# someone-in-somewhere/multimodal_rag

Hardware: AMD Instinct MI355X
Metric: chunks embedded/sec + queries/sec top_k=5 over 1M×768 at 1/2/4/8 GPUs (higher is better)
Workload: dtype f16

## Files before the change

multimodal_rag_amd/csrc/encoder.hip:

```cpp
#include "mmrag_internal.h"
#include "tile_dma.h"

#include <atomic>
#include <chrono>
#include <type_traits>

#include <limits.h>
#include <stdlib.h>

using namespace mmrag;

namespace mmrag_impl {

constexpr float NEG_INF_F = -__builtin_inff();
typedef _Float16 half2_t __attribute__((ext_vector_type(2)));
__device__ inline float2 h2f(half2_t t) { return make_float2((float)t[0], (float)t[1]); }
__device__ inline half2_t f2h(float a, float b) {
    half2_t r;
    r[0] = (_Float16)a;
    r[1] = (_Float16)b;
    return r;
}

__device__ inline float wave_sum(float v) {
// ... 795 lines not shown
            const int c = wave + i * NWAVES;
            vreg[i] = make_uint4(0, 0, 0, 0);
            if (c < CH && k0 + lane < len) vreg[i] = *(const uint4 *)(Vp + (size_t)(k0 + lane) * ld + c * 8);
        }
    };
    auto store_tile_from = [&](int buf, const uint4(&kreg)[K_ITERS], const uint4(&vreg)[V_ITERS]) {
        char *kb = smem + buf * (K_BYTES + V_BYTES);
        char *vb = kb + K_BYTES;
#pragma unroll
        for (int i = 0; i < K_ITERS; ++i) {
            const int idx = threadIdx.x + i * NT;
            const int key = idx / CH, c = idx % CH;
            if (idx < KT * CH) {
                const int cs = DH == 64 ? (c ^ ((key >> 1) & 7)) : (c ^ ((key >> 2) & 3));
                *(uint4 *)(kb + key * KROW + cs * 16) = kreg[i];
            }
        }
#pragma unroll
        for (int i = 0; i < V_ITERS; ++i) {
            const int c = wave + i * NWAVES;
            if (c < CH) {
                const unsigned w[4] = {vreg[i].x, vreg[i].y, vreg[i].z, vreg[i].w};
#pragma unroll
                for (int e = 0; e < 8; ++e) {
                    const unsigned short bits = (unsigned short)(w[e >> 1] >> ((e & 1) * 16));
                    *(unsigned short *)(vb + (c * 8 + e) * VROW + lane * 2) = bits;
                }
            }
        }
    };

    f32x16_t o[NDB];
#pragma unroll
    for (int d = 0; d < NDB; ++d)
#pragma unroll
        for (int j = 0; j < 16; ++j) o[d][j] = 0.f;
    float m_run = NEG_INF_F, l_run = 0.f;

    auto load_tile = [&](int kt) { load_tile_into(kt, kreg0, vreg0); };
    auto store_tile = [&](int buf) { store_tile_from(buf, kreg0, vreg0); };
    if constexpr (RESIDENT) {
        uint4 kr[MAXT - 1][K_ITERS], vr[MAXT - 1][V_ITERS];
        load_tile(0);
#pragma unroll
        for (int t = 1; t < MAXT; ++t)
            if (t < n_tiles) load_tile_into(t, kr[t - 1], vr[t - 1]);
        store_tile(0);
#pragma unroll
        for (int t = 1; t < MAXT; ++t)
            if (t < n_tiles) store_tile_from(t, kr[t - 1], vr[t - 1]);
    } else {
        load_tile(0);
        store_tile(0);
    }
    __syncthreads();
    for (int kt = 0; kt < n_tiles; ++kt) {
        const int buf = RESIDENT ? kt : (kt & 1);
        if constexpr (!RESIDENT)
            if (kt + 1 < n_tiles) load_tile(kt + 1);
        const char *kb = smem + buf * (K_BYTES + V_BYTES);
        const char *vb = kb + K_BYTES;

        f32x16_t s[2];
#pragma unroll
        for (int b = 0; b < 2; ++b) {
#pragma unroll
            for (int j = 0; j < 16; ++j) s[b][j] = 0.f;
            const int key = b * 32 + r32;
#pragma unroll
            for (int ks = 0; ks < NQK; ++ks) {
                const int c = 2 * ks + hh;
                const int cs = DH == 64 ? (c ^ ((key >> 1) & 7)) : (c ^ ((key >> 2) & 3));
                const half8_t kf = *(const half8_t *)(kb + key * KROW + cs * 16);
                s[b] = __builtin_amdgcn_mfma_f32_32x32x16_f16(kf, qf[ks], s[b], 0, 0, 0);
            }
        }
        const int k0 = kt * KT;
        const bool edge = (k0 + KT > len) || (causal && k0 + KT - 1 > q_tile0 + wave * 32);
        if (edge) {
#pragma unroll
            for (int b = 0; b < 2; ++b)
#pragma unroll
                for (int j = 0; j < 16; ++j) {
                    const int key = k0 + b * 32 + (j & 3) + 8 * (j >> 2) + 4 * hh;
                    const bool ok = key < len && (!causal || key <= qi);
                    s[b][j] = ok ? s[b][j] : NEG_INF_F;
                }
        }
        float m_tile = NEG_INF_F;
#pragma unroll
        for (int b = 0; b < 2; ++b)
#pragma unroll
            for (int j = 0; j < 16; j += 2) m_tile = fmaxf(m_tile, fmaxf(s[b][j], s[b][j + 1]));
        m_tile = fmaxf(m_tile, __shfl_xor(m_tile, 32));
        const float m_new = fmaxf(m_run, m_tile);
        const float m_use = m_new == NEG_INF_F ? 0.f : m_new;
        const float c2 = scale * 1.4426950408889634f;
        const float mc = m_use * c2;
        const float alpha = __builtin_amdgcn_exp2f(m_run * c2 - mc);
        float psum = 0.f;
        half8_t pf[2][2];
#pragma unroll
        for (int b = 0; b < 2; ++b)
#pragma unroll
            for (int j = 0; j < 16; ++j) {
                const float pv = __builtin_amdgcn_exp2f(fmaf(s[b][j], c2, -mc));
                psum += pv;
                pf[b][j >> 3][j & 7] = (_Float16)pv;
            }
        l_run = l_run * alpha + psum;
        m_run = m_new;
#pragma unroll
        for (int d = 0; d < NDB; ++d)
#pragma unroll
            for (int j = 0; j < 16; ++j) o[d][j] *= alpha;
#pragma unroll
        for (int d = 0; d < NDB; ++d) {
            const char *vrow = vb + (d * 32 + r32) * VROW;
#pragma unroll
            for (int b = 0; b < 2; ++b)
#pragma unroll
                for (int st = 0; st < 2; ++st) {
                    const int kk = b * 32 + st * 16 + 4 * hh;
                    const half4_t lo = *(const half4_t *)(vrow + kk * 2);
                    const half4_t hi = *(const half4_t *)(vrow + (kk + 8) * 2);
                    half8_t vf;
#pragma unroll
                    for (int i = 0; i < 4; ++i) {
                        vf[i] = lo[i];
                        vf[4 + i] = hi[i];
                    }
                    o[d] = __builtin_amdgcn_mfma_f32_32x32x16_f16(vf, pf[b][st], o[d], 0, 0, 0);
                }
        }
        if constexpr (!RESIDENT) {
            if (kt + 1 < n_tiles) store_tile(buf ^ 1);
            __syncthreads();
        }
    }

    const float l_tot = l_run + __shfl_xor(l_run, 32);
    const float inv = l_tot > 0.f ? 1.0f / l_tot : 0.f;
    if (qi < len) {
        _Float16 *dst = ctx + (size_t)(seq0 + qi) * H + head * DH;
#pragma unroll
        for (int d = 0; d < NDB; ++d)
#pragma unroll
            for (int g = 0; g < 4; ++g) {
                half4_t v;
#pragma unroll
                for (int i = 0; i < 4; ++i) v[i] = (_Float16)(o[d][4 * g + i] * inv);
                *(half4_t *)(dst + d * 32 + 8 * g + 4 * hh) = v;
            }
    }
#endif
}

template <typename OutT>
__global__ __launch_bounds__(256) void pool_norm_kernel(const _Float16 *__restrict__ x,
                                                         const int *__restrict__ cu_seqlens,
                                                         const int *__restrict__ sel, OutT *__restrict__ out,
                                                         int H, int pool, int normalize) {
    __shared__ float red[4];
    const int b = blockIdx.x;
    const int s0 = cu_seqlens[b], s1 = cu_seqlens[b + 1];
    float vals[4];
    float sq = 0.f;
#pragma unroll
    for (int i = 0; i < 4; ++i) {
        const int c = threadIdx.x + i * 256;
        float v = 0.f;
        if (c < H) {
            if (pool == 0) {
                for (int t = s0; t < s1; ++t) v += (float)x[(size_t)t * H + c];
                const float cnt = (float)(s1 - s0);
                v = v / fmaxf(cnt, 1e-9f);
            } else {
                const int t = pool == 1 ? s0 : s0 + sel[b];
                v = (float)x[(size_t)t * H + c];
            }
        }
        vals[i] = v;
        sq += v * v;
    }
    sq = wave_sum(sq);
    if ((threadIdx.x & 63) == 0) red[threadIdx.x >> 6] = sq;
    __syncthreads();
    const float nrm = sqrtf(red[0] + red[1] + red[2] + red[3]);
    const float inv = normalize ? 1.0f / fmaxf(nrm, 1e-12f) : 1.0f;
#pragma unroll
    for (int i = 0; i < 4; ++i) {
        const int c = threadIdx.x + i * 256;
        if (c < H) out[(size_t)b * H + c] = (OutT)(vals[i] * inv);
    }
}

__global__ __launch_bounds__(256) void patchify_kernel(const void *__restrict__ pixels, int kind,
                                                        _Float16 *__restrict__ patches, int B, int IMG, int P) {
    const int G = IMG / P, NP = G * G, PK = 3 * P * P, CH = PK / 8;
    const long long total = (long long)B * NP * CH;
    const long long i = (long long)blockIdx.x * blockDim.x + threadIdx.x;
    if (i >= total) return;
    const int ch = (int)(i % CH);
    const long long prow = i / CH;
    const int pidx = (int)(prow % NP), b = (int)(prow / NP);
    const int e0 = ch * 8;
    const int c = e0 / (P * P), ph = (e0 / P) % P, pw = e0 % P;
    const int y = (pidx / G) * P + ph, x0 = (pidx % G) * P + pw;
    half8_t o;
    if (kind == MMRAG_PIXELS_F16_CHW) {
        o = *(const half8_t *)((const _Float16 *)pixels + (((size_t)b * 3 + c) * IMG + y) * IMG + x0);
    } else {
        const float mean[3] = {0.48145466f, 0.4578275f, 0.40821073f};
        const float stdv[3] = {0.26862954f, 0.26130258f, 0.27577711f};
        const unsigned char *src = (const unsigned char *)pixels + (((size_t)b * IMG + y) * IMG + x0) * 3 + c;
#pragma unroll
        for (int e = 0; e < 8; ++e) o[e] = (_Float16)(((float)src[e * 3] / 255.0f - mean[c]) / stdv[c]);
    }
    *(half8_t *)(patches + (size_t)prow * PK + e0) = o;
}

__global__ __launch_bounds__(256) void vit_assemble_ln_kernel(const _Float16 *__restrict__ emb,
                                                               const _Float16 *__restrict__ cls,
                                                               const _Float16 *__restrict__ pos,
                                                               const float *__restrict__ g, const float *__restrict__ b,
                                                               _Float16 *__restrict__ out, int T, int H, int S,
                                                               float eps) {
    const int lane = threadIdx.x & 63;
    const int row = blockIdx.x * 4 + (threadIdx.x >> 6);
    if (row >= T) return;
    const int t = row % S, img = row / S;
    const _Float16 *src = t == 0 ? cls : emb + ((size_t)img * (S - 1) + (t - 1)) * H;
    ln_row<2>(src, out + (size_t)row * H, g, b, H, eps, lane, pos + (size_t)t * H);
}

__global__ __launch_bounds__(256) void normalize_rows_kernel(const _Float16 *__restrict__ x, float *__restrict__ out,
                                                              int B, int D) {
    const int lane = threadIdx.x & 63;
    const int row = blockIdx.x * 4 + (threadIdx.x >> 6);
    if (row >= B) return;
    float sq = 0.f;
    for (int c = lane; c < D; c += 64) {
        const float v = (float)x[(size_t)row * D + c];
        sq += v * v;
    }
    const float inv = 1.0f / fmaxf(sqrtf(wave_sum(sq)), 1e-12f);
    for (int c = lane; c < D; c += 64) out[(size_t)row * D + c] = (float)x[(size_t)row * D + c] * inv;
}

template <int NWC>
__global__ __launch_bounds__(64 * NWC) void linear_small_kernel(const LinearParams p) {
#if defined(__HIP_DEVICE_COMPILE__)
    __shared__ float part[NWC][16][64];
    const int lane = threadIdx.x & 63;
    const int wave = threadIdx.x >> 6;
    const int r32 = lane & 31, h = lane >> 5;
    const int f0 = blockIdx.x * 32;
    const int kw = p.K / NWC;
    const int k_lo = wave * kw;
    const int fr = f0 + r32 < p.N ? f0 + r32 : p.N - 1;
    const _Float16 *wrow = (const _Float16 *)p.wt + (size_t)fr * p.K + k_lo + 8 * h;
    for (int t0 = 0; t0 < p.M; t0 += 32) {
        const int tr = t0 + r32 < p.M ? t0 + r32 : p.M - 1;
        const _Float16 *xrow = (const _Float16 *)p.x + (size_t)tr * p.K + k_lo + 8 * h;
        f32x16_t acc;
#pragma unroll
        for (int j = 0; j < 16; ++j) acc[j] = 0.0f;
        for (int k = 0; k < kw; k += 64) {
            half8_t a[4], b[4];
#pragma unroll
            for (int s_ = 0; s_ < 4; ++s_) {
                const bool in = k + 16 * s_ < kw;
                a[s_] = *(const half8_t *)(wrow + (in ? k + 16 * s_ : 0));
                b[s_] = *(const half8_t *)(xrow + (in ? k + 16 * s_ : 0));
            }
#pragma unroll
            for (int s_ = 0; s_ < 4; ++s_)
                if (k + 16 * s_ < kw) acc = __builtin_amdgcn_mfma_f32_32x32x16_f16(a[s_], b[s_], acc, 0, 0, 0);
        }
        if (t0 > 0) __syncthreads();
#pragma unroll
        for (int j = 0; j < 16; ++j) part[wave][j][lane] = acc[j];
        __syncthreads();
        const int g = wave & 3;
        const int t = t0 + r32;
        const int f = f0 + 8 * g + 4 * h;
        float v[4] = {0.f, 0.f, 0.f, 0.f};
        if (wave < 4) {
#pragma unroll
            for (int w = 0; w < NWC; ++w)
#pragma unroll
                for (int i = 0; i < 4; ++i) v[i] += part[w][4 * g + i][lane];
        }
        if (wave < 4 && t < p.M && f < p.N) {
            if (p.bias != nullptr) {
                const float4 bv = *(const float4 *)(p.bias + f);
                v[0] += bv.x, v[1] += bv.y, v[2] += bv.z, v[3] += bv.w;
            }
            half4_t o;
            if (p.act == MMRAG_ACT_GELU) {
#pragma unroll
                for (int i = 0; i < 4; ++i) o[i] = (_Float16)act_apply<MMRAG_ACT_GELU>(v[i]);
            } else if (p.act == MMRAG_ACT_QUICK_GELU) {
#pragma unroll
                for (int i = 0; i < 4; ++i) o[i] = (_Float16)act_apply<MMRAG_ACT_QUICK_GELU>(v[i]);
            } else {
// ... 136 lines not shown
    float2 *ln_stats_out = nullptr;
    const float2 *res_stats = nullptr;
    const float *res_gamma = nullptr, *res_beta = nullptr;
};

static bool takes_small16_kernel(long long M, int K, bool ln_in) {
    if (M > 64 || (debug_flags() & (DBG_LINEAR_NO_SMALL | DBG_LINEAR_SMALL32))) return false;
    if (ln_in) return K == 384 || K == 512 || K == 768 || K == 1024;
    return K == 384 || K == 512 || K == 768 || K == 1024 || K == 1536 || K == 2048 || K == 3072;
}

int launch_linear(const void *x, int M, int K, const void *wt, int N, const float *bias, int act,
                  const void *resid, void *out, hipStream_t s, const SmallNorms *norms = nullptr) {
    LinearParams p;
    p.ln_gamma = p.ln_beta = nullptr, p.ln_eps = 0.f, p.ln_stats_out = nullptr;
    p.res_stats = nullptr, p.res_gamma = p.res_beta = nullptr;
    if (norms != nullptr) {
        if (!takes_small16_kernel(M, K, norms->ln_gamma != nullptr)) {
            set_error("linear: folded LayerNorm needs the 16-feature single-query kernel (M=%d K=%d)", M, K);
            return MMRAG_EUNSUPPORTED;
        }
        p.ln_gamma = norms->ln_gamma, p.ln_beta = norms->ln_beta, p.ln_eps = norms->ln_eps, p.ln_stats_out = norms->ln_stats_out;
        p.res_stats = norms->res_stats, p.res_gamma = norms->res_gamma, p.res_beta = norms->res_beta;
    }
    p.x = (const char *)x;
    p.wt = (const char *)wt;
    p.bias = bias;
    p.resid = (const _Float16 *)resid;
    p.out = (_Float16 *)out;
    p.M = M, p.N = N, p.K = K, p.act = act;
    const unsigned dbg = debug_flags();
    p.xcd_order = (dbg & DBG_LINEAR_PLAIN) ? 0 : 1;
    p.dbg = dbg;
    if (M <= 64 && !(dbg & (DBG_LINEAR_NO_SMALL | DBG_LINEAR_SMALL32))) {
        const unsigned g16 = (unsigned)((N + 15) / 16);
        bool done = true;
        if (p.ln_gamma != nullptr) {
            if (K == 384) linear_small16_kernel<12, 1, true><<<g16, 768, 0, s>>>(p);
            else if (K == 512) linear_small16_kernel<16, 1, true><<<g16, 1024, 0, s>>>(p);
            else if (K == 768) linear_small16_kernel<12, 2, true><<<g16, 768, 0, s>>>(p);
            else linear_small16_kernel<16, 2, true><<<g16, 1024, 0, s>>>(p);
        } else if (K == 384) linear_small16_kernel<12, 1><<<g16, 768, 0, s>>>(p);
        else if (K == 512) linear_small16_kernel<16, 1><<<g16, 1024, 0, s>>>(p);
        else if (K == 768) linear_small16_kernel<12, 2><<<g16, 768, 0, s>>>(p);
        else if (K == 1024) linear_small16_kernel<16, 2><<<g16, 1024, 0, s>>>(p);
        else if (K == 1536) linear_small16_kernel<16, 3><<<g16, 1024, 0, s>>>(p);
        else if (K == 2048) linear_small16_kernel<16, 4><<<g16, 1024, 0, s>>>(p);
        else if (K == 3072) linear_small16_kernel<16, 6><<<g16, 1024, 0, s>>>(p);
        else done = false;
        if (done) return MMRAG_OK;
    }
    if (M <= 64 && (K / 4) % 16 == 0 && !(dbg & DBG_LINEAR_NO_SMALL)) {
        const unsigned g = (unsigned)((N + 31) / 32);
        if (K % 256 == 0) linear_small_kernel<16><<<g, 1024, 0, s>>>(p);
        else if (K % 128 == 0) linear_small_kernel<8><<<g, 512, 0, s>>>(p);
        else linear_small_kernel<4><<<g, 256, 0, s>>>(p);
        return MMRAG_OK;
    }
    const int cus = num_cus();
    const long long big_tiles = (long long)((M + 255) / 256) * ((N + 255) / 256);
    const long long tiles_f = (N + 255) / 256;
    const bool big_pays = (double)N >= 0.65 * (double)(tiles_f * 256);
    if (big_tiles >= cus && big_pays) {
        if (dbg & DBG_LINEAR_PLAIN)
            linear_kernel<256, 256, 4, 4, 2><<<(unsigned)big_tiles, 1024, 0, s>>>(p);
        else if (K >= 128 && N % 2 == 0 && !(dbg & DBG_LINEAR_NO_PERSIST)) {
            const unsigned grid = (unsigned)(big_tiles < cus ? big_tiles : cus);
            if (!(dbg & DBG_LINEAR_MFMA32) && N % 4 == 0) linear_persistent_kernel<2, 4, 16><<<grid, 512, 0, s>>>(p, (int)big_tiles, (int)tiles_f);
            else linear_persistent_kernel<2, 4, 32><<<grid, 512, 0, s>>>(p, (int)big_tiles, (int)tiles_f);
        } else
            linear_kernel<256, 256, 4, 4, 2, true><<<(unsigned)big_tiles, 1024, 0, s>>>(p);
    } else {
        const long long tiles = (long long)((M + 127) / 128) * ((N + 127) / 128);
        if ((dbg & DBG_LINEAR_TILE64) || (!(dbg & DBG_LINEAR_TILE128) && tiles < cus / 2)) {
            const long long t64 = (long long)((M + 63) / 64) * ((N + 63) / 64);
            linear_kernel<64, 64, 1, 1, 2, true><<<(unsigned)t64, 64, 0, s>>>(p);
            return MMRAG_OK;
        }
        linear_kernel<128, 128, 2, 2, 2, true><<<(unsigned)tiles, 256, 0, s>>>(p);
    }
    return MMRAG_OK;
}

}
using namespace mmrag_impl;

static std::atomic<long long> g_last_forward_us{0};

extern "C" {

int mmrag_linear_f16(const void *x, int64_t M, int K, const void *wt, int N, const float *bias, int act,
                     const void *resid, void *out, void *stream) {
    MMRAG_CHECK_ARG(x && wt && out, "linear: null pointer");
    MMRAG_CHECK_ARG(M > 0 && M < INT_MAX && N > 0 && K > 0, "linear: bad shape M=%lld N=%d K=%d", (long long)M, N, K);
    MMRAG_CHECK_ARG(K % 64 == 0, "linear: K=%d must be a multiple of 64 (128-byte fp16 slabs)", K);
    MMRAG_CHECK_ARG(N % 4 == 0, "linear: N=%d must be a multiple of 4", N);
    MMRAG_CHECK_ARG(act >= 0 && act <= 2, "linear: bad activation %d", act);
    MMRAG_CHECK_ARG(((uintptr_t)x % 16) == 0 && ((uintptr_t)wt % 16) == 0 && ((uintptr_t)out % 8) == 0 &&
                        ((uintptr_t)resid % 8) == 0 && ((uintptr_t)bias % 16) == 0,
                    "linear: misaligned pointer");
    launch_linear(x, (int)M, K, wt, N, bias, act, resid, out, (hipStream_t)stream);
    MMRAG_CHECK_HIP(hipGetLastError());
    return MMRAG_OK;
}

int mmrag_internal_linear_f16_norms(const void *x, int64_t M, int K, const void *wt, int N, const float *bias, int act,
                                    const void *resid, void *out, const float *ln_gamma, const float *ln_beta,
                                    float ln_eps, float *ln_stats_out, const float *res_stats, const float *res_gamma,
                                    const float *res_beta, void *stream) {
    MMRAG_CHECK_ARG(x && wt && out, "linear_norms: null pointer");
    MMRAG_CHECK_ARG(M > 0 && M <= 64 && N > 0 && N % 4 == 0, "linear_norms: bad shape M=%lld N=%d", (long long)M, N);
    MMRAG_CHECK_ARG(act >= 0 && act <= 2, "linear_norms: bad activation %d", act);
    MMRAG_CHECK_ARG((ln_gamma == nullptr) == (ln_beta == nullptr), "linear_norms: ln_gamma / ln_beta both or neither");
    MMRAG_CHECK_ARG(res_stats == nullptr || (resid && res_gamma && res_beta), "linear_norms: res_stats needs resid, res_gamma, res_beta");
    MMRAG_CHECK_ARG(((uintptr_t)x % 16) == 0 && ((uintptr_t)wt % 16) == 0 && ((uintptr_t)out % 8) == 0 &&
                        ((uintptr_t)resid % 8) == 0 && ((uintptr_t)bias % 16) == 0 && ((uintptr_t)ln_gamma % 16) == 0 &&
                        ((uintptr_t)ln_beta % 16) == 0 && ((uintptr_t)ln_stats_out % 8) == 0 &&
                        ((uintptr_t)res_stats % 8) == 0 && ((uintptr_t)res_gamma % 16) == 0 &&
                        ((uintptr_t)res_beta % 16) == 0,
                    "linear_norms: misaligned pointer");
    SmallNorms n;
    n.ln_gamma = ln_gamma, n.ln_beta = ln_beta, n.ln_eps = ln_eps, n.ln_stats_out = (float2 *)ln_stats_out;
    n.res_stats = (const float2 *)res_stats, n.res_gamma = res_gamma, n.res_beta = res_beta;
    const int st = launch_linear(x, (int)M, K, wt, N, bias, act, resid, out, (hipStream_t)stream, &n);
    if (st != MMRAG_OK) return st;
    MMRAG_CHECK_HIP(hipGetLastError());
    return MMRAG_OK;
}

int mmrag_layernorm_f16(const void *x, void *out, const float *gamma, const float *beta, int64_t T, int H,
                        float eps, void *stream) {
    MMRAG_CHECK_ARG(x && out && gamma && beta, "layernorm: null pointer");
    MMRAG_CHECK_ARG(T > 0 && H > 0 && H % 8 == 0 && H <= 1024, "layernorm: bad shape T=%lld H=%d (H % 8 == 0, <= 1024)", (long long)T, H);
    MMRAG_CHECK_ARG(((uintptr_t)x % 16) == 0 && ((uintptr_t)out % 16) == 0 && ((uintptr_t)gamma % 16) == 0 && ((uintptr_t)beta % 16) == 0, "layernorm: pointers must be 16-byte aligned");
    layernorm_kernel<<<(unsigned)((T + 3) / 4), 256, 0, (hipStream_t)stream>>>(
        (const _Float16 *)x, (_Float16 *)out, gamma, beta, (int)T, H, eps);
    MMRAG_CHECK_HIP(hipGetLastError());
    return MMRAG_OK;
}

int mmrag_embed_ln_f16(const int32_t *ids, const int32_t *pos_ids, const void *tok, const void *pos,
                       const void *type0, const float *gamma, const float *beta, void *out, int64_t T, int H,
                       int vocab, int max_pos, float eps, void *stream) {
    MMRAG_CHECK_ARG(ids && pos_ids && tok && pos && out, "embed_ln: null pointer");
    MMRAG_CHECK_ARG((gamma == nullptr) == (beta == nullptr), "embed_ln: gamma/beta must both be given or both null");
    MMRAG_CHECK_ARG(T > 0 && H > 0 && H % 8 == 0 && H <= 1024, "embed_ln: bad shape T=%lld H=%d", (long long)T, H);
    embed_ln_kernel<<<(unsigned)((T + 3) / 4), 256, 0, (hipStream_t)stream>>>(
        ids, pos_ids, (const _Float16 *)tok, (const _Float16 *)pos, (const _Float16 *)type0, gamma, beta,
        (_Float16 *)out, (int)T, H, vocab, max_pos, eps);
    MMRAG_CHECK_HIP(hipGetLastError());
    return MMRAG_OK;
}

int mmrag_attention_f16(const void *qkv, const int32_t *cu_seqlens, void *ctx, int B, int max_len, int H,
                        int n_heads, int causal, void *stream) {
    MMRAG_CHECK_ARG(qkv && cu_seqlens && ctx, "attention: null pointer");
    MMRAG_CHECK_ARG(B > 0 && max_len > 0 && n_heads > 0 && H % n_heads == 0, "attention: bad shape");
    const int dh = H / n_heads;
    MMRAG_CHECK_ARG(dh == 32 || dh == 64, "attention: head dim %d unsupported (32 or 64)", dh);
    MMRAG_CHECK_ARG(((uintptr_t)qkv % 16) == 0 && ((uintptr_t)ctx % 8) == 0, "attention: misaligned pointer");
    const dim3 grid((unsigned)((max_len + 127) / 128), (unsigned)n_heads, (unsigned)B);
    const float scale = 1.0f / sqrtf((float)dh);
    if (dh == 64 && max_len <= 256 && max_len > 128 && !(debug_flags() & DBG_ATTENTION_STREAMED)) {
        const dim3 grid8((unsigned)((max_len + 255) / 256), (unsigned)n_heads, (unsigned)B);
        attention_kernel<64, 2, true, 8><<<grid8, 512, 0, (hipStream_t)stream>>>((const _Float16 *)qkv, cu_seqlens,
                                                                                 (_Float16 *)ctx, H, scale, causal);
    } else if (dh == 64 && max_len > 256 && max_len <= 512 && !(debug_flags() & DBG_ATTENTION_STREAMED)) {
        const dim3 grid16((unsigned)((max_len + 511) / 512), (unsigned)n_heads, (unsigned)B);
        attention_kernel<64, 1, true, 16, 8><<<grid16, 1024, 0, (hipStream_t)stream>>>((const _Float16 *)qkv, cu_seqlens,
                                                                                       (_Float16 *)ctx, H, scale, causal);
    } else if (dh == 64)
        attention_kernel<64, 3><<<grid, 256, 0, (hipStream_t)stream>>>((const _Float16 *)qkv, cu_seqlens,
                                                                       (_Float16 *)ctx, H, scale, causal);
    else if (max_len <= 256 && max_len > 128 && !(debug_flags() & DBG_ATTENTION_STREAMED)) {
        const dim3 grid8((unsigned)((max_len + 255) / 256), (unsigned)n_heads, (unsigned)B);
        attention_kernel<32, 2, true, 8><<<grid8, 512, 0, (hipStream_t)stream>>>((const _Float16 *)qkv, cu_seqlens,
                                                                                 (_Float16 *)ctx, H, scale, causal);
    } else
        attention_kernel<32, 3><<<grid, 256, 0, (hipStream_t)stream>>>((const _Float16 *)qkv, cu_seqlens,
                                                                       (_Float16 *)ctx, H, scale, causal);
    MMRAG_CHECK_HIP(hipGetLastError());
    return MMRAG_OK;
}

int mmrag_pool_normalize_f16(const void *x, const int32_t *cu_seqlens, const int32_t *sel, float *out, int B,
                             int H, int pool, int normalize, void *stream) {
    MMRAG_CHECK_ARG(x && cu_seqlens && out, "pool: null pointer");
    MMRAG_CHECK_ARG(B > 0 && H > 0 && H <= 1024, "pool: bad shape B=%d H=%d", B, H);
    MMRAG_CHECK_ARG(pool >= 0 && pool <= 2 && (pool != 2 || sel), "pool: bad mode %d", pool);
    pool_norm_kernel<float><<<(unsigned)B, 256, 0, (hipStream_t)stream>>>((const _Float16 *)x, cu_seqlens, sel, out, H,
                                                                         pool, normalize);
    MMRAG_CHECK_HIP(hipGetLastError());
    return MMRAG_OK;
}


static size_t align256(size_t x) { return (x + 255) / 256 * 256; }

static size_t hm_elems(const mmrag_encoder_desc *d, int64_t T, int B) {
    size_t n = (size_t)T * (size_t)d->intermediate;
    if (d->patch > 0 && d->image > 0) {
        const size_t g = (size_t)(d->image / d->patch);
        const size_t patches = (size_t)B * g * g * 3 * (size_t)d->patch * (size_t)d->patch;
        if (patches > n) n = patches;
    }
    return n;
}

size_t mmrag_encoder_workspace_bytes(const mmrag_encoder_desc *d, int64_t T, int B) {
    if (!d || T <= 0 || B <= 0) return 0;
    const size_t H = (size_t)d->hidden, I = (size_t)d->intermediate;
    size_t bytes = 0;
    bytes += 2 * align256((size_t)T * H * 2);
    bytes += align256((size_t)T * 3 * H * 2);
    bytes += align256((size_t)T * H * 2);
    bytes += align256(hm_elems(d, T, B) * 2);
    bytes += 2 * align256((size_t)B * (H > (size_t)d->out_dim ? H : (size_t)d->out_dim) * 2);
    bytes += 2 * align256(64 * 8);
    return bytes + 256;
}

struct EncBuffers {
    void *x, *y, *qkv, *ctx, *hm, *pooled, *proj;
    float2 *stats_a, *stats_b;
};

static int carve(const mmrag_encoder_desc *d, int64_t T, int B, void *workspace, size_t workspace_bytes,
                 EncBuffers *b) {
    const size_t need = mmrag_encoder_workspace_bytes(d, T, B);
    if (!workspace || workspace_bytes < need) {
        set_error("encoder_forward: workspace %zu bytes < required %zu", workspace_bytes, need);
        return MMRAG_EWORKSPACE;
    }
    const size_t H = (size_t)d->hidden, Tz = (size_t)T;
    char *p = (char *)(((uintptr_t)workspace + 255) / 256 * 256);
    auto take = [&](size_t bytes) { char *r = p; p += align256(bytes); return (void *)r; };
    b->x = take(Tz * H * 2), b->y = take(Tz * H * 2), b->qkv = take(Tz * 3 * H * 2), b->ctx = take(Tz * H * 2);
    b->hm = take(hm_elems(d, T, B) * 2);
    const size_t pd = (size_t)(d->hidden > d->out_dim ? d->hidden : d->out_dim);
    b->pooled = take((size_t)B * pd * 2), b->proj = take((size_t)B * pd * 2);
    b->stats_a = (float2 *)take(64 * 8), b->stats_b = (float2 *)take(64 * 8);
    return MMRAG_OK;
}

#define RUN(call) do { if ((st = (call)) != MMRAG_OK) return st; } while (0)

static int encoder_body(const mmrag_encoder_desc *d, const void *const *lw, const EncBuffers &b,
                        const int32_t *cu_seqlens, const int32_t *sel, int64_t T, int B, int max_len, float *out,
                        void *stream) {
    const int H = d->hidden, I = d->intermediate, L = d->n_layers;
    void *x = b.x, *y = b.y, *qkv = b.qkv, *ctx = b.ctx, *hm = b.hm;
    int st;
    const int causal = d->causal;
    hipStream_t s = (hipStream_t)stream;
    const bool folded_ln = d->arch == MMRAG_ARCH_BERT && !(debug_flags() & DBG_ENCODER_LN_PASSES) &&
                           takes_small16_kernel(T, H, true) && takes_small16_kernel(T, I, false);
    if (folded_ln) {
        const float *g_prev = nullptr, *b_prev = nullptr;
        for (int l = 0; l < L; ++l, lw += 12) {
            const float *bqkv = (const float *)lw[1], *bo = (const float *)lw[3];
            const float *g1 = (const float *)lw[4], *b1n = (const float *)lw[5];
            const float *bi = (const float *)lw[7], *b2 = (const float *)lw[9];
            SmallNorms nq, no, n1, n2;
            if (l > 0) {
                nq.ln_gamma = g_prev, nq.ln_beta = b_prev, nq.ln_eps = d->ln_eps, nq.ln_stats_out = b.stats_b;
                no.res_stats = b.stats_b, no.res_gamma = g_prev, no.res_beta = b_prev;
            }
            RUN(launch_linear(x, (int)T, H, lw[0], 3 * H, bqkv, MMRAG_ACT_NONE, nullptr, qkv, s, &nq));
            RUN(mmrag_attention_f16(qkv, cu_seqlens, ctx, B, max_len, H, d->n_heads, causal, stream));
            RUN(launch_linear(ctx, (int)T, H, lw[2], H, bo, MMRAG_ACT_NONE, x, y, s, &no));
            n1.ln_gamma = g1, n1.ln_beta = b1n, n1.ln_eps = d->ln_eps, n1.ln_stats_out = b.stats_a;
            RUN(launch_linear(y, (int)T, H, lw[6], I, bi, d->act, nullptr, hm, s, &n1));
            n2.res_stats = b.stats_a, n2.res_gamma = g1, n2.res_beta = b1n;
            RUN(launch_linear(hm, (int)T, I, lw[8], H, b2, MMRAG_ACT_NONE, y, x, s, &n2));
            g_prev = (const float *)lw[10], b_prev = (const float *)lw[11];
        }
        MMRAG_CHECK_HIP(hipGetLastError());
        RUN(mmrag_layernorm_f16(x, y, g_prev, b_prev, T, H, d->ln_eps, stream));
        return mmrag_pool_normalize_f16(y, cu_seqlens, sel, out, B, H, d->pool, d->normalize, stream);
    }
    for (int l = 0; l < L; ++l, lw += 12) {
        const float *bqkv = (const float *)lw[1], *bo = (const float *)lw[3];
        const float *g1 = (const float *)lw[4], *b1n = (const float *)lw[5];
        const float *bi = (const float *)lw[7], *b2 = (const float *)lw[9];
        const float *g2 = (const float *)lw[10], *b2n = (const float *)lw[11];
        if (d->arch == MMRAG_ARCH_BERT) {
            RUN(mmrag_linear_f16(x, T, H, lw[0], 3 * H, bqkv, MMRAG_ACT_NONE, nullptr, qkv, stream));
            RUN(mmrag_attention_f16(qkv, cu_seqlens, ctx, B, max_len, H, d->n_heads, causal, stream));
            RUN(mmrag_linear_f16(ctx, T, H, lw[2], H, bo, MMRAG_ACT_NONE, x, y, stream));
            RUN(mmrag_layernorm_f16(y, x, g1, b1n, T, H, d->ln_eps, stream));
            RUN(mmrag_linear_f16(x, T, H, lw[6], I, bi, d->act, nullptr, hm, stream));
            RUN(mmrag_linear_f16(hm, T, I, lw[8], H, b2, MMRAG_ACT_NONE, x, y, stream));
            RUN(mmrag_layernorm_f16(y, x, g2, b2n, T, H, d->ln_eps, stream));
        } else {
            RUN(mmrag_layernorm_f16(x, y, g1, b1n, T, H, d->ln_eps, stream));
            RUN(mmrag_linear_f16(y, T, H, lw[0], 3 * H, bqkv, MMRAG_ACT_NONE, nullptr, qkv, stream));
            RUN(mmrag_attention_f16(qkv, cu_seqlens, ctx, B, max_len, H, d->n_heads, causal, stream));
            RUN(mmrag_linear_f16(ctx, T, H, lw[2], H, bo, MMRAG_ACT_NONE, x, x, stream));
            RUN(mmrag_layernorm_f16(x, y, g2, b2n, T, H, d->ln_eps, stream));
            RUN(mmrag_linear_f16(y, T, H, lw[6], I, bi, d->act, nullptr, hm, stream));
            RUN(mmrag_linear_f16(hm, T, I, lw[8], H, b2, MMRAG_ACT_NONE, x, x, stream));
        }
    }
    if (d->arch == MMRAG_ARCH_BERT) {
        RUN(mmrag_pool_normalize_f16(x, cu_seqlens, sel, out, B, H, d->pool, d->normalize, stream));
    } else {
        RUN(mmrag_layernorm_f16(x, y, (const float *)lw[0], (const float *)lw[1], T, H, d->ln_eps, stream));
        pool_norm_kernel<_Float16><<<(unsigned)B, 256, 0, s>>>((const _Float16 *)y, cu_seqlens, sel,
                                                               (_Float16 *)b.pooled, H, d->pool, 0);
        MMRAG_CHECK_HIP(hipGetLastError());
        RUN(mmrag_linear_f16(b.pooled, B, H, lw[2], d->out_dim, nullptr, MMRAG_ACT_NONE, nullptr, b.proj, stream));
        normalize_rows_kernel<<<(unsigned)((B + 3) / 4), 256, 0, s>>>((const _Float16 *)b.proj, out, B, d->out_dim);
        MMRAG_CHECK_HIP(hipGetLastError());
    }
    return MMRAG_OK;
// ... 178 lines not shown
```

multimodal_rag_amd/csrc/mmrag_internal.h:

```cpp
#pragma once
#include <hip/hip_runtime.h>
#include <stdint.h>
#include <stdio.h>
#include <stdarg.h>

#include "../../include/mmrag.h"

namespace mmrag {

void set_error(const char *fmt, ...);

inline int esize(int dtype) { return dtype == MMRAG_F32 ? 4 : (dtype == MMRAG_F8E4M3 ? 1 : 2); }

constexpr size_t align_up(size_t x, size_t a) { return (x + a - 1) / a * a; }

template <int DT>
struct ElemTag {
    static constexpr int value = DT;
};
template <typename F>
inline auto with_elem_type(int dtype, F &&f) {
    if (dtype == MMRAG_F32) return f(ElemTag<MMRAG_F32>{});
    if (dtype == MMRAG_F16) return f(ElemTag<MMRAG_F16>{});
    return f(ElemTag<MMRAG_BF16>{});
}

#define MMRAG_CHECK_ARG(cond, ...)            \
    do {                                      \
        if (!(cond)) {                        \
            mmrag::set_error(__VA_ARGS__);    \
            return MMRAG_EINVAL;              \
        }                                     \
    } while (0)

#define MMRAG_CHECK_HIP(expr)                                                     \
    do {                                                                          \
        hipError_t e_ = (expr);                                                   \
        if (e_ != hipSuccess) {                                                   \
            mmrag::set_error("%s failed: %s", #expr, hipGetErrorString(e_));      \
            return MMRAG_EHIP;                                                    \
        }                                                                         \
    } while (0)

int num_cus();

unsigned debug_flags();
constexpr unsigned DBG_LINEAR_PLAIN = 1u, DBG_LINEAR_NO_SMALL = 2u, DBG_LINEAR_NO_PERSIST = 4u;
constexpr unsigned DBG_LINEAR_DROP_STORES = 8u, DBG_LINEAR_SKIP_EPILOGUE = 16u;
constexpr unsigned DBG_LINEAR_X_SAME = 128u;
constexpr unsigned DBG_LINEAR_MFMA32 = 8192u;
constexpr unsigned DBG_LINEAR_SMALL32 = 256u;
constexpr unsigned DBG_ENCODER_LN_PASSES = 512u;
constexpr unsigned DBG_ATTENTION_STREAMED = 4096u;
constexpr unsigned DBG_LINEAR_TILE64 = 1024u, DBG_LINEAR_TILE128 = 2048u;

}

extern "C" {
int mmrag_internal_join_tile(int64_t T, int64_t id, int64_t *ti, int64_t *tj);
int mmrag_internal_join_slot_tile(int64_t T, int64_t slot, int64_t *ti, int64_t *tj);
}

namespace mmrag_impl {
size_t cls_head_workspace_bytes(int B, int H, int NL);
int cls_head_counters(int B);
int *cls_head_counter_ptr(void *ws, int B, int H, int NL);
int launch_cls_head_f32(const float *cls, const float *wp, const float *bp, const float *wc, const float *bc, float *out,
                        int B, int H, int NL, void *ws, hipStream_t s);
}
```

multimodal_rag_amd/csrc/tile_dma.h:

```cpp
#pragma once
#include <hip/hip_runtime.h>
#include <stdint.h>

#include "../../include/mmrag.h"

namespace mmrag_impl {

typedef _Float16 half8_t __attribute__((ext_vector_type(8)));
typedef _Float16 half4_t __attribute__((ext_vector_type(4)));
typedef __bf16 bf16x8_t __attribute__((ext_vector_type(8)));
typedef float f32x4_t __attribute__((ext_vector_type(4)));
typedef float f32x16_t __attribute__((ext_vector_type(16)));
typedef __attribute__((address_space(3))) void *lds_ptr_t;

template <int DT>
struct FragType;
template <>
struct FragType<MMRAG_F16> {
    using T = half8_t;
    __device__ static __forceinline__ f32x4_t mfma_16x16x32(T a, T b, f32x4_t c) {
        return __builtin_amdgcn_mfma_f32_16x16x32_f16(a, b, c, 0, 0, 0);
    }
};
template <>
struct FragType<MMRAG_BF16> {
    using T = bf16x8_t;
    __device__ static __forceinline__ f32x4_t mfma_16x16x32(T a, T b, f32x4_t c) {
        return __builtin_amdgcn_mfma_f32_16x16x32_bf16(a, b, c, 0, 0, 0);
    }
};

constexpr int SLAB = 128;

template <int N>
__device__ inline void wait_vmcnt() {
    asm volatile("s_waitcnt vmcnt(%0)" ::"n"(N) : "memory");
}

template <int LOADS, int MAXITEMS>
__device__ inline void wait_items(int items) {
    if constexpr (MAXITEMS >= 3) {
        if (items >= 3) {
            wait_vmcnt<3 * LOADS>();
            return;
        }
    }
    if constexpr (MAXITEMS >= 2) {
        if (items >= 2) {
            wait_vmcnt<2 * LOADS>();
            return;
        }
    }
    if constexpr (MAXITEMS >= 1) {
        if (items >= 1) {
            wait_vmcnt<LOADS>();
            return;
        }
    }
    wait_vmcnt<0>();
}

__device__ inline __amdgpu_buffer_rsrc_t make_rsrc(const void *base, unsigned bytes) {
    return __builtin_amdgcn_make_buffer_rsrc(const_cast<void *>(base), 0, bytes, 0x00020000);
}

__device__ inline unsigned dma_src_offset(int piece, int lane, unsigned row_bytes) {
    const int row = piece * 8 + (lane >> 3);
    return (unsigned)row * row_bytes + (unsigned)(((lane & 7) ^ ((row >> 1) & 7)) * 16);
}

__device__ inline void dma_piece(__amdgpu_buffer_rsrc_t rsrc, char *lds_tile, int piece, unsigned src_off) {
    __builtin_amdgcn_raw_ptr_buffer_load_lds(rsrc, (lds_ptr_t)(lds_tile + piece * 1024), 16, src_off, 0, 0, 0);
}

__device__ inline int frag_offset(int row, int chunk) { return row * SLAB + ((chunk ^ ((row >> 1) & 7)) * 16); }


}
```

Baseline: 661,000.

## Add ring-buffered attention kernel with DMA K/V staging and transposed LDS reads

```diff
diff --git a/multimodal_rag_amd/csrc/encoder.hip b/multimodal_rag_amd/csrc/encoder.hip
--- a/multimodal_rag_amd/csrc/encoder.hip
+++ b/multimodal_rag_amd/csrc/encoder.hip
@@ -971,6 +971,244 @@
                 for (int i = 0; i < 4; ++i) v[i] = (_Float16)(o[d][4 * g + i] * inv);
                 *(half4_t *)(dst + d * 32 + 8 * g + 4 * hh) = v;
             }
+    }
+#endif
+}
+
+#if defined(MMRAG_ATTN_DEV)
+#define MMRAG_ATTN_STAMP_PARAM , unsigned long long *__restrict__ stamps, int n_stamps
+#else
+#define MMRAG_ATTN_STAMP_PARAM
+#endif
+template <int DH, bool PARTNER>
+__global__ __launch_bounds__(512, 2) void attention_ring_kernel(const _Float16 *__restrict__ qkv,
+                                                                const int *__restrict__ cu_seqlens,
+                                                                _Float16 *__restrict__ ctx, int H, int n_heads,
+                                                                float scale MMRAG_ATTN_STAMP_PARAM) {
+#if defined(__HIP_DEVICE_COMPILE__)
+    static_assert(DH == 32 || DH == 64, "head dim");
+    constexpr int KT = 64;
+    constexpr int NH = 64 / DH;
+    constexpr int NQK = DH / 16;
+    constexpr int NDB = DH / 32;
+    constexpr int NSTAGE = 4;
+    constexpr int AHEAD = PARTNER ? 2 : 3;
+    constexpr int TILE = KT * SLAB, STAGE = 2 * TILE;
+    __shared__ __attribute__((aligned(1024))) char smem[NSTAGE * STAGE];
+
+    const int lane = threadIdx.x & 63;
+    const int wave = __builtin_amdgcn_readfirstlane(threadIdx.x >> 6);
+    const int r32 = lane & 31;
+    const int hh = lane >> 5;
+    const int head0 = blockIdx.y * NH;
+    const int seq0 = cu_seqlens[blockIdx.z];
+    const int len = cu_seqlens[blockIdx.z + 1] - seq0;
+    const int q_tile0 = blockIdx.x * 256;
+    if (q_tile0 >= len) return;
+    const int ld = 3 * H;
+    const unsigned row_b = (unsigned)ld * 2u;
+    const int heads_here = n_heads - head0 < NH ? n_heads - head0 : NH;
+    const bool active = q_tile0 + wave * 32 < len;
+
+    const int qi = q_tile0 + wave * 32 + r32;
+    half8_t qf[NH][NQK];
+#pragma unroll
+    for (int hd = 0; hd < NH; ++hd)
+#pragma unroll
+        for (int ks = 0; ks < NQK; ++ks) {
+            if (qi < len && hd < heads_here)
+                qf[hd][ks] = *(const half8_t *)(qkv + (size_t)(seq0 + qi) * ld + (head0 + hd) * DH + ks * 16 + hh * 8);
+            else
+#pragma unroll
+                for (int i = 0; i < 8; ++i) qf[hd][ks][i] = (_Float16)0.f;
+        }
+
+    asm volatile("" ::: "memory");
+
+    const int n_tiles = (len + KT - 1) / KT;
+    const char *kbase = (const char *)(qkv + (size_t)seq0 * ld + H + head0 * DH);
+    const unsigned extent = (unsigned)(len - 1) * row_b + (unsigned)(heads_here * DH * 2);
+    const __amdgpu_buffer_rsrc_t k_rs = make_rsrc(kbase, extent), v_rs = make_rsrc(kbase + (size_t)H * 2, extent);
+    const unsigned k_src = dma_src_offset(wave, lane, row_b), v_src = dma_src_offset_tr(wave, lane, row_b);
+    auto issue = [&](int t) {
+        char *st = smem + (t % NSTAGE) * STAGE;
+        const unsigned tile_off = (unsigned)(t * KT) * row_b;
+        dma_piece(k_rs, st, wave, k_src + tile_off);
+        dma_piece(v_rs, st + TILE, wave, v_src + tile_off);
+    };
+
+    f32x16_t o[NH][NDB];
+    float m_run[NH], l_run[NH], alpha[NH];
+    half8_t pf[NH][2][2];
+#pragma unroll
+    for (int hd = 0; hd < NH; ++hd) {
+        m_run[hd] = NEG_INF_F;
+        l_run[hd] = 0.f;
+        alpha[hd] = 1.f;
+#pragma unroll
+        for (int d = 0; d < NDB; ++d)
+#pragma unroll
+            for (int j = 0; j < 16; ++j) o[hd][d][j] = 0.f;
+    }
+    const float c2 = scale * 1.4426950408889634f;
+
+    auto scores = [&](int kt, int hd) {
+        const char *kb = smem + (kt % NSTAGE) * STAGE;
+        f32x16_t s[2];
+#pragma unroll
+        for (int b = 0; b < 2; ++b) {
+#pragma unroll
+            for (int j = 0; j < 16; ++j) s[b][j] = 0.f;
+            const int key = b * 32 + r32;
+#pragma unroll
+            for (int ks = 0; ks < NQK; ++ks) {
+                const half8_t kf = *(const half8_t *)(kb + frag_offset(key, hd * (DH / 8) + 2 * ks + hh));
+                s[b] = __builtin_amdgcn_mfma_f32_32x32x16_f16(kf, qf[hd][ks], s[b], 0, 0, 0);
+            }
+        }
+        const int k0 = kt * KT;
+        if (k0 + KT > len) {
+#pragma unroll
+            for (int b = 0; b < 2; ++b)
+#pragma unroll
+                for (int j = 0; j < 16; ++j) {
+                    const int key = k0 + b * 32 + (j & 3) + 8 * (j >> 2) + 4 * hh;
+                    s[b][j] = key < len ? s[b][j] : NEG_INF_F;
+                }
+        }
+        float m_tile = NEG_INF_F;
+#pragma unroll
+        for (int b = 0; b < 2; ++b)
+#pragma unroll
+            for (int j = 0; j < 16; j += 2) m_tile = fmaxf(fmaxf(m_tile, s[b][j]), s[b][j + 1]);
+        m_tile = fmaxf(m_tile, __shfl_xor(m_tile, 32));
+        const float m_new = fmaxf(m_run[hd], m_tile);
+        const float m_use = m_new == NEG_INF_F ? 0.f : m_new;
+        const float mc = m_use * c2;
+        alpha[hd] = __builtin_amdgcn_exp2f(m_run[hd] * c2 - mc);
+        float psum = 0.f;
+#pragma unroll
+        for (int b = 0; b < 2; ++b)
+#pragma unroll
+            for (int j = 0; j < 16; ++j) {
+                const float pv = __builtin_amdgcn_exp2f(fmaf(s[b][j], c2, -mc));
+                psum += pv;
+                pf[hd][b][j >> 3][j & 7] = (_Float16)pv;
+            }
+        l_run[hd] = l_run[hd] * alpha[hd] + psum;
+        m_run[hd] = m_new;
+    };
+    unsigned v_tr[NH * NDB];
+#pragma unroll
+    for (int i = 0; i < NH * NDB; ++i) v_tr[i] = lds_address(smem) + (unsigned)(tr_lane_offset(lane, i) + 4 * hh * SLAB);
+    auto context = [&](int kt, int hd) {
+#pragma unroll
+        for (int d = 0; d < NDB; ++d) {
+            const unsigned vcol = v_tr[hd * NDB + d] + (unsigned)((kt % NSTAGE) * STAGE);
+            half4_t lo[2][2], hi[2][2];
+#define MMRAG_TR(b_, s_)                                                                   \
+    lo[b_][s_] = ds_read_tr16_async<TILE + ((b_) * 32 + (s_) * 16) * SLAB>(vcol);          \
+    hi[b_][s_] = ds_read_tr16_async<TILE + ((b_) * 32 + (s_) * 16 + 8) * SLAB>(vcol)
+            MMRAG_TR(0, 0);
+            MMRAG_TR(0, 1);
+            MMRAG_TR(1, 0);
+            MMRAG_TR(1, 1);
+#undef MMRAG_TR
+#pragma unroll
+            for (int j = 0; j < 16; ++j) o[hd][d][j] *= alpha[hd];
+            tr_wait<6>(lo[0][0], hi[0][0]);
+            tr_wait<4>(lo[0][1], hi[0][1]);
+            tr_wait<2>(lo[1][0], hi[1][0]);
+            tr_wait<0>(lo[1][1], hi[1][1]);
+#pragma unroll
+            for (int b = 0; b < 2; ++b)
+#pragma unroll
+                for (int s2 = 0; s2 < 2; ++s2) {
+                    half8_t vf;
+#pragma unroll
+                    for (int i = 0; i < 4; ++i) {
+                        vf[i] = lo[b][s2][i];
+                        vf[4 + i] = hi[b][s2][i];
+                    }
+                    o[hd][d] = __builtin_amdgcn_mfma_f32_32x32x16_f16(vf, pf[hd][b][s2], o[hd][d], 0, 0, 0);
+                }
+        }
+    };
+
+    const bool late = PARTNER && wave >= 4;
+    if constexpr (PARTNER)
+        if (wave >= 4) __builtin_amdgcn_s_setprio(1);
+    int issued = 0;
+#pragma unroll
+    for (; issued < AHEAD; ++issued) issue(issued);
+#pragma unroll
+    for (int hd = 0; hd < NH; ++hd)
+#pragma unroll
+        for (int ks = 0; ks < NQK; ++ks) asm volatile("" : "+v"(qf[hd][ks]));
+#if defined(MMRAG_ATTN_DEV)
+    const unsigned long long t0c = __builtin_amdgcn_s_memtime(), t0r = __builtin_amdgcn_s_memrealtime();
+#endif
+    for (int kt = 0; kt < n_tiles; ++kt) {
+        asm volatile("s_waitcnt lgkmcnt(0)" ::: "memory");
+        wait_items<2, AHEAD - 1>(issued - kt - 1);
+        __builtin_amdgcn_s_barrier();
+        if (issued < n_tiles) {
+            issue(issued);
+            ++issued;
+        }
+        if (active) {
+            if (late) {
+                if (kt > 0) {
+#pragma unroll
+                    for (int hd = 0; hd < NH; ++hd) context(kt - 1, hd);
+                }
+#pragma unroll
+                for (int hd = 0; hd < NH; ++hd) scores(kt, hd);
+            } else {
+#pragma unroll
+                for (int hd = 0; hd < NH; ++hd) {
+                    scores(kt, hd);
+                    context(kt, hd);
+                }
+            }
+        }
+    }
+    if (active && late) {
+#pragma unroll
+        for (int hd = 0; hd < NH; ++hd) context(n_tiles - 1, hd);
+    }
+    wait_vmcnt<0>();
+#if defined(MMRAG_ATTN_DEV)
+    {
+        const int wg = (blockIdx.z * gridDim.y + blockIdx.y) * gridDim.x + blockIdx.x;
+        if (stamps != nullptr && threadIdx.x == 0 && wg < n_stamps) {
+            stamps[2 * wg] = __builtin_amdgcn_s_memtime() - t0c;
+            stamps[2 * wg + 1] = __builtin_amdgcn_s_memrealtime() - t0r;
+        }
+    }
+#endif
+
+    float inv[NH];
+#pragma unroll
+    for (int hd = 0; hd < NH; ++hd) {
+        const float l_tot = l_run[hd] + __shfl_xor(l_run[hd], 32);
+        inv[hd] = l_tot > 0.f ? 1.0f / l_tot : 0.f;
+    }
+    if (qi < len) {
+#pragma unroll
+        for (int hd = 0; hd < NH; ++hd) {
+            if (hd >= heads_here) break;
+            _Float16 *dst = ctx + (size_t)(seq0 + qi) * H + (head0 + hd) * DH;
+#pragma unroll
+            for (int d = 0; d < NDB; ++d)
+#pragma unroll
+                for (int g = 0; g < 4; ++g) {
+                    half4_t v;
+#pragma unroll
+                    for (int i = 0; i < 4; ++i) v[i] = (_Float16)(o[hd][d][4 * g + i] * inv[hd]);
+                    *(half4_t *)(dst + d * 32 + 8 * g + 4 * hh) = v;
+                }
+        }
     }
 #endif
 }
@@ -1413,6 +1651,19 @@
     return MMRAG_OK;
 }
 
+static const bool g_attn_v1_env = [] {
+    const char *e = getenv("MMRAG_ATTN_V1");
+    return e != nullptr && atoi(e) != 0;
+}();
+#if defined(MMRAG_ATTN_DEV)
+static unsigned long long *g_attn_stamps = nullptr;
+static int g_attn_n_stamps = 0;
+extern "C" void mmrag_internal_attention_stamps(void *buf, int n_workgroups) {
+    g_attn_stamps = (unsigned long long *)buf;
+    g_attn_n_stamps = n_workgroups;
+}
+#endif
+
 int mmrag_attention_f16(const void *qkv, const int32_t *cu_seqlens, void *ctx, int B, int max_len, int H,
                         int n_heads, int causal, void *stream) {
     MMRAG_CHECK_ARG(qkv && cu_seqlens && ctx, "attention: null pointer");
@@ -1422,6 +1673,29 @@
     MMRAG_CHECK_ARG(((uintptr_t)qkv % 16) == 0 && ((uintptr_t)ctx % 8) == 0, "attention: misaligned pointer");
     const dim3 grid((unsigned)((max_len + 127) / 128), (unsigned)n_heads, (unsigned)B);
     const float scale = 1.0f / sqrtf((float)dh);
+    const unsigned dbg = debug_flags();
+    const bool v1 = g_attn_v1_env || (dbg & (DBG_ATTENTION_V1 | DBG_ATTENTION_STREAMED));
+    if (!causal && !v1 && max_len <= 512 && ((dh == 64 && max_len > 128 && max_len <= 256) || (dbg & DBG_ATTENTION_RING_ALL))) {
+        const int nh_wg = 64 / dh;
+        const dim3 gridr((unsigned)((max_len + 255) / 256), (unsigned)((n_heads + nh_wg - 1) / nh_wg), (unsigned)B);
+        const bool partner = (dbg & DBG_ATTENTION_PARTNER) != 0;
+#if defined(MMRAG_ATTN_DEV)
+#define MMRAG_ATTN_STAMP_ARGS , g_attn_stamps, g_attn_n_stamps
+#else
+#define MMRAG_ATTN_STAMP_ARGS
+#endif
+#define MMRAG_LAUNCH_RING(DH_, P_)                                                                              \
+    attention_ring_kernel<DH_, P_><<<gridr, 512, 0, (hipStream_t)stream>>>((const _Float16 *)qkv, cu_seqlens,  \
+                                                                           (_Float16 *)ctx, H, n_heads, scale  \
+                                                                               MMRAG_ATTN_STAMP_ARGS)
+        if (dh == 64 && partner) MMRAG_LAUNCH_RING(64, true);
+        else if (dh == 64) MMRAG_LAUNCH_RING(64, false);
+        else if (partner) MMRAG_LAUNCH_RING(32, true);
+        else MMRAG_LAUNCH_RING(32, false);
+#undef MMRAG_LAUNCH_RING
+        MMRAG_CHECK_HIP(hipGetLastError());
+        return MMRAG_OK;
+    }
     if (dh == 64 && max_len <= 256 && max_len > 128 && !(debug_flags() & DBG_ATTENTION_STREAMED)) {
         const dim3 grid8((unsigned)((max_len + 255) / 256), (unsigned)n_heads, (unsigned)B);
         attention_kernel<64, 2, true, 8><<<grid8, 512, 0, (hipStream_t)stream>>>((const _Float16 *)qkv, cu_seqlens,
diff --git a/multimodal_rag_amd/csrc/mmrag_internal.h b/multimodal_rag_amd/csrc/mmrag_internal.h
--- a/multimodal_rag_amd/csrc/mmrag_internal.h
+++ b/multimodal_rag_amd/csrc/mmrag_internal.h
@@ -52,6 +52,7 @@
 constexpr unsigned DBG_LINEAR_SMALL32 = 256u;
 constexpr unsigned DBG_ENCODER_LN_PASSES = 512u;
 constexpr unsigned DBG_ATTENTION_STREAMED = 4096u;
+constexpr unsigned DBG_ATTENTION_V1 = 16384u, DBG_ATTENTION_RING_ALL = 32768u, DBG_ATTENTION_PARTNER = 65536u;
 constexpr unsigned DBG_LINEAR_TILE64 = 1024u, DBG_LINEAR_TILE128 = 2048u;
 
 }
diff --git a/multimodal_rag_amd/csrc/tile_dma.h b/multimodal_rag_amd/csrc/tile_dma.h
--- a/multimodal_rag_amd/csrc/tile_dma.h
+++ b/multimodal_rag_amd/csrc/tile_dma.h
@@ -75,5 +75,33 @@
 
 __device__ inline int frag_offset(int row, int chunk) { return row * SLAB + ((chunk ^ ((row >> 1) & 7)) * 16); }
 
+__device__ inline int tr_swizzle(int row) { return ((row >> 1) & 1) << 2; }
+
+__device__ inline unsigned dma_src_offset_tr(int piece, int lane, unsigned row_bytes) {
+    const int row = piece * 8 + (lane >> 3);
+    return (unsigned)row * row_bytes + (unsigned)(((lane & 7) ^ tr_swizzle(row)) * 16);
+}
+
+__device__ inline int tr_lane_offset(int lane, int blk32) {
+    const int q = (lane >> 2) & 3, p = lane & 3, g1 = (lane >> 4) & 1;
+    const int chunk = 4 * blk32 + 2 * g1 + (p >> 1);
+    return q * SLAB + ((chunk ^ tr_swizzle(q)) * 16) + 8 * (p & 1);
+}
+
+__device__ inline unsigned lds_address(const char *p) {
+    return (unsigned)(uintptr_t)(__attribute__((address_space(3))) const char *)p;
+}
+template <int OFFSET>
+__device__ inline half4_t ds_read_tr16_async(unsigned lds_addr) {
+    static_assert(OFFSET >= 0 && OFFSET < 65536, "ds immediate offset");
+    half4_t r;
+    asm volatile("ds_read_b64_tr_b16 %0, %1 offset:%2" : "=v"(r) : "v"(lds_addr), "n"(OFFSET) : "memory");
+    return r;
+}
+template <int N>
+__device__ inline void tr_wait(half4_t &a, half4_t &b) {
+    asm volatile("s_waitcnt lgkmcnt(%2)" : "+v"(a), "+v"(b) : "n"(N));
+}
+
 
 }
```

New measurement: 662,800 (median of 5 runs). No clear change (+0.3%).
